# ORNL/HydraGNN

Hardware: NVIDIA H100
Metric: atoms_per_sec_training_step (higher is better)
Workload: dtype tf32

## Files before the change

hydragnn_b200/ops.py:

```python
import os

import torch
from torch.autograd.function import once_differentiable

from . import _lib

ACT_CODES = {None: 0, "none": 0, "relu": 1, "silu": 2, "tanh": 3, "sigmoid": 4, "lrelu": 5, "elu": 6, "selu": 7}
POOL_CODES = {"add": 0, "sum": 0, "mean": 1, "max": 2}


def _stream():
    return torch.cuda.current_stream().cuda_stream


def _p(t):
    return None if t is None else t.data_ptr()


def _chk(t, dtype=torch.float32):
    if t is None:
        return None
    if not t.is_cuda:
        raise RuntimeError("hydragnn_b200 ops need CUDA tensors (no CPU fallback on the hot path)")
    if t.dtype != dtype:
# ... 2 lines not shown


def _ws(nbytes, device):
    return torch.empty(max(int(nbytes), 16), dtype=torch.uint8, device=device)


class Csr:
    __slots__ = ("idx", "rowptr", "perm", "n")

    def __init__(self, idx, rowptr, perm, n):
        self.idx, self.rowptr, self.perm, self.n = idx, rowptr, perm, n


def csr_build(index64, n):
    index64 = _chk(index64, torch.int64)
    e = index64.numel()
    dev = index64.device
    idx32 = torch.empty(e, dtype=torch.int32, device=dev)
    rowptr = torch.empty(n + 1, dtype=torch.int32, device=dev)
    perm = torch.empty(e, dtype=torch.int32, device=dev)
    ws = _ws(_lib.query("hgb_csr_workspace_bytes", e, n), dev)
    _lib.call("hgb_csr_build", _p(index64), e, n, _p(idx32), _p(rowptr), _p(perm), _p(guard_flag(dev)), _p(ws), _stream())
    return Csr(idx32, rowptr, perm, n)


def csr_build_grouped(index64, n, node_ptr, edge_ptr, g):
    index64 = _chk(index64, torch.int64)
    e = index64.numel()
    dev = index64.device
    idx32 = torch.empty(e, dtype=torch.int32, device=dev)
    rowptr = torch.empty(n + 1, dtype=torch.int32, device=dev)
    perm = torch.empty(e, dtype=torch.int32, device=dev)
    ws = _ws(_lib.query("hgb_csr_grouped_workspace_bytes", e, n), dev)
    _lib.call("hgb_csr_build_grouped", _p(index64), e, n, _p(node_ptr), _p(edge_ptr), int(g), _p(idx32), _p(rowptr), _p(perm),
              _p(guard_flag(dev)), _p(ws), _stream())
    return Csr(idx32, rowptr, perm, n)


class EdgePlan:

    def __init__(self, edge_index, num_nodes, col_rowptr=None, graph_ptr=None):
        ei = _chk(edge_index, torch.int64)
        self.num_nodes, self.num_edges = int(num_nodes), int(ei.shape[1])
        if col_rowptr is not None and graph_ptr is not None and GROUPED_CSR:
            self.by_row = csr_build_grouped(ei[0], self.num_nodes, graph_ptr, col_rowptr, graph_ptr.numel() - 1)
        else:
            self.by_row = csr_build(ei[0], self.num_nodes)
        if col_rowptr is not None:
            self.by_col = Csr(ei[1].to(torch.int32), col_rowptr, torch.arange(self.num_edges, dtype=torch.int32, device=ei.device),
                              self.num_nodes)
        else:
            self.by_col = csr_build(ei[1], self.num_nodes)
        self.row, self.col = self.by_row.idx, self.by_col.idx
        self._nbr = {}

    def nbr(self, which):
        if which not in self._nbr:
            idx, perm = (self.col, self.by_row.perm) if which == "row" else (self.row, self.by_col.perm)
            out = torch.empty_like(perm)
            _lib.call("hgb_gather_i32", _p(idx), _p(perm), perm.numel(), _p(out), _stream())
            self._nbr[which] = out
        return self._nbr[which]


def graph_ptr_from_batch(batch, num_graphs):
    return csr_build(batch, num_graphs)


def exclusive_scan(x):
    x = _chk(x, torch.int32)
    out = torch.empty(x.numel() + 1, dtype=torch.int32, device=x.device)
    ws = _ws(_lib.query("hgb_exclusive_scan_workspace_bytes", x.numel()), x.device)
    _lib.call("hgb_exclusive_scan_i32", _p(x), _p(out), x.numel(), _p(ws), _stream())
    return out


GUARD_EDGE_COUNT = 1
GUARD_BAD_INDEX = 2
_GUARD = {}


def guard_flag(device):
    key = torch.device(device).index if torch.device(device).index is not None else torch.cuda.current_device()
    if key not in _GUARD:
        _GUARD[key] = torch.zeros(1, dtype=torch.int32, device=torch.device("cuda", key))
    return _GUARD[key]


def expect_count(value_i32, expected, bit=GUARD_EDGE_COUNT):
    _lib.call("hgb_expect_i32", _p(value_i32), int(expected), int(bit), _p(guard_flag(value_i32.device)), _stream())


def check_guard(device=None):
    dev = torch.device("cuda", torch.cuda.current_device()) if device is None else torch.device(device)
    word = int(guard_flag(dev).item())
    if word:
        guard_flag(dev).zero_()
        what = []
        if word & GUARD_EDGE_COUNT:
            what.append("a neighbour build produced a different edge count than the one the step was captured with")
        if word & GUARD_BAD_INDEX:
            what.append("an index vector had entries outside [0, n)")
        raise RuntimeError("hydragnn_b200 device guard tripped: " + "; ".join(what))


def raw_gather(x, idx32):
    x = _chk(x)
# ... 559 lines not shown
        gv = torch.empty_like(vec)
        _lib.call("hgb_edge_geom_bwd", _p(vec), _p(ln), ctx.eps, _p(_chk(g_vec)), _p(_chk(g_len)), _p(_chk(g_unit)),
                  plan.num_edges, _p(gv), _stream())
        g_pos = g_shift = None
        if ctx.needs_input_grad[0]:
            g_pos = raw_segment_sum(gv, plan.by_col.rowptr, plan.by_col.perm, plan.num_nodes) - \
                raw_segment_sum(gv, plan.by_row.rowptr, plan.by_row.perm, plan.num_nodes)
        if ctx.needs_input_grad[1]:
            g_shift = gv
        return g_pos, g_shift, None, None


class PainnEdgeEmbedFn(torch.autograd.Function):

    @staticmethod
    def forward(ctx, unit, ln, num_radial, cutoff):
        e = unit.shape[0]
        epack = torch.empty(e, 12, dtype=unit.dtype, device=unit.device)
        _lib.call("hgb_painn_edge_embed_fwd", _p(unit), _p(ln), e, num_radial, float(cutoff), _p(epack), _stream())
        ctx.save_for_backward(unit, ln)
        ctx.r, ctx.cutoff = num_radial, float(cutoff)
        return epack

    @staticmethod
    @once_differentiable
    def backward(ctx, g_epack):
        unit, ln = ctx.saved_tensors
        e = unit.shape[0]
        g_unit = torch.empty_like(unit)
        g_len = torch.empty_like(ln)
        _lib.call("hgb_painn_edge_embed_bwd", _p(unit), _p(ln), _p(_chk(g_epack)), e, ctx.r, ctx.cutoff, _p(g_unit), _p(g_len), _stream())
        return g_unit, g_len, None, None


class PainnMessageFn(torch.autograd.Function):

    @staticmethod
    def forward(ctx, phi, s, v, epack, wf, bf, efilt, plan, rec_row=None):
        n, f = s.shape
        r = wf.shape[1]
        phi, s, v = _chk(phi), _chk(s), _chk(v)
        s_out, v_out = torch.empty_like(s), torch.empty_like(v)
        agg = plan.by_row
        _lib.call("hgb_painn_message_fwd", _p(phi), _p(s), _p(v), _p(agg.rowptr), _p(agg.perm), _p(plan.nbr("row")), _p(epack),
                  _p(rec_row), _p(_chk(wf)), _p(_chk(bf)), _p(_chk(efilt)), n, f, r, _p(s_out), _p(v_out), _stream())
        ctx.save_for_backward(phi, v, epack, wf, bf, efilt)
        ctx.plan, ctx.use_rec = plan, rec_row is not None
        return s_out, v_out

    @staticmethod
    @once_differentiable
    def backward(ctx, gs_out, gv_out):
        phi, v, epack, wf, bf, efilt = ctx.saved_tensors
        plan = ctx.plan
        n, f = gs_out.shape
        r = wf.shape[1]
        gs_out, gv_out = _chk(gs_out), _chk(gv_out)
        need_edge = ctx.needs_input_grad[3]
        gphi, gv = torch.empty_like(phi), torch.empty_like(v)
        gwf, gbf = torch.empty_like(wf), torch.empty_like(bf)
        cpl = 2 if (f >= 64 and f % 2 == 0) else 1
        multi = f > 32 * cpl
        g_epack = (torch.zeros_like(epack) if multi else torch.empty_like(epack)) if need_edge else None
        g_ef = torch.empty_like(efilt) if efilt is not None else None
        nbytes = _lib.query("hgb_painn_message_bwd_workspace_bytes", n, f, r)
        ws = _ws(nbytes, phi.device)
        src = plan.by_col
        rec_col = None
        if ctx.use_rec:
            cache = plan.__dict__.setdefault("_rec_col", {})
            key = epack.data_ptr()
            if key not in cache:
                cache.clear()
                cache[key] = painn_edge_records(epack, plan, "col")
            rec_col = cache[key]
        _lib.call("hgb_painn_message_bwd", _p(gs_out), _p(gv_out), _p(phi), _p(v), _p(src.rowptr), _p(src.perm), _p(plan.nbr("col")),
                  _p(epack), _p(rec_col), _p(wf), _p(bf), _p(efilt), n, f, r, _p(gphi), _p(gv), _p(gwf), _p(gbf), _p(g_epack), _p(g_ef),
                  _p(ws), nbytes, _stream())
        return gphi, gs_out, gv, g_epack, gwf, gbf, g_ef, None, None


def painn_edge_records(epack, plan, which):
    csr = plan.by_row if which == "row" else plan.by_col
    rec = torch.empty(plan.num_edges, 16, dtype=epack.dtype, device=epack.device)
    _lib.call("hgb_painn_edge_records", _p(epack.detach()), _p(csr.perm), _p(plan.nbr(which)), plan.num_edges, _p(rec), _stream())
    return rec


def raw_linear(x2, w, b, code=0, param=0.0, want_z=False):
    m, k = x2.shape
    n = w.shape[0]
    y = torch.empty(m, n, dtype=x2.dtype, device=x2.device)
    z = torch.empty_like(y) if want_z else None
    if gemm3_ok(x2, w, y, m, n, k, False, True):
        _lib.call("hgb_gemm3", _p(x2), _p(w), _p(y), m, n, k, 0, 1, x2.stride(0), w.stride(0), n, 0, _p(b), code, float(param), _p(z), None,
                  _stream())
        return y, z
    _lib.call("hgb_linear_fwd", _p(x2), _p(w), _p(b), m, n, k, x2.stride(0), w.stride(0), code, float(param), _p(y), _p(z), _stream())
    return y, z


def raw_act_bwd(dy, y, z, code, param=0.0):
    dz = torch.empty_like(dy)
    _lib.call("hgb_act_bwd", _p(dy), _p(y), _p(z), dy.numel(), code, float(param), _p(dz), _stream())
    return dz


class PainnUpdateFn(torch.autograd.Function):

    @staticmethod
    def forward(ctx, s, v, uw, ub, vw, vb, w1, b1, w2, b2, last):
        n, f = s.shape
        s, v = _chk(s), _chk(v)
        w1, b1, w2, b2 = [_chk(t) for t in (w1, b1, w2, b2)]
        v2 = v.reshape(3 * n, f)
        wuv, buv = torch.cat([uw, vw], dim=0).contiguous(), torch.cat([ub, vb], dim=0).contiguous()
        y_uv, _ = linear_fwd_dispatch(v2, wuv, buv)
        uv, vv, ld = y_uv, y_uv[:, f:], 2 * f
        mlp_in = torch.empty(n, 2 * f, dtype=s.dtype, device=s.device)
        _lib.call("hgb_painn_update_pre_fwd", _p(vv), ld, _p(s), n, f, _p(mlp_in), _stream())
        h, z1, deriv = linear_fwd_dispatch_ex(mlp_in, w1, b1, ACT_CODES["silu"], 0.0, want_z=True, z_deriv=True)
        a, _ = linear_fwd_dispatch(h, w2, b2)
        ctx.z1_code = ACT_DERIV if deriv else ACT_CODES["silu"]
        s_out = torch.empty_like(s)
        v_out = None if last else torch.empty_like(v)
        _lib.call("hgb_painn_update_post_fwd", _p(a), _p(uv), _p(vv), ld, _p(s), _p(v), n, f, int(last), _p(s_out), _p(v_out), _stream())
        ctx.save_for_backward(v2, y_uv, mlp_in, z1, h, a, wuv, w1, w2)
        ctx.last = bool(last)
        ctx.tc = _TC["enabled"]
        ctx.leaves = ([uw, ub, vw, vb], [w1, b1], [w2, b2])
        if last:
            return s_out, s_out.new_zeros(0)
# ... 682 lines not shown
```

hydragnn_b200/stacks.py:

```python
import os

import torch
import torch.nn.functional as F
from torch import nn

from . import ops
from .ops import GatherRows, LinearAct, MatMul, SegmentSum


def activation_function_selection(name):
    table = {"relu": nn.ReLU, "selu": nn.SELU, "elu": nn.ELU, "sigmoid": nn.Sigmoid,
             "lrelu_01": lambda: nn.LeakyReLU(0.1), "lrelu_025": lambda: nn.LeakyReLU(0.25),
             "lrelu_05": lambda: nn.LeakyReLU(0.5)}
    if name == "prelu":
        raise ValueError("activation 'prelu' (a learnable slope) is not supported by the b200 engine")
    if name not in table:
        raise ValueError("Unknown activation function: " + str(name))
    return table[name]()


def _act_code(mod):
    if isinstance(mod, nn.ReLU):
        return "relu", 0.0
    if isinstance(mod, nn.SiLU):
# ... 154 lines not shown
            return self._forward_fused(x, coord, plan, edge_shifts, higher_order, cache)
        if higher_order:
            vec = GatherRows.apply(coord, plan.by_col) - GatherRows.apply(coord, plan.by_row)
            if edge_shifts is not None:
                vec = vec + edge_shifts
            radial = torch.linalg.norm(vec, dim=-1, keepdim=True)
            coord_diff = vec / (radial + 1.0)
        else:
            _, radial, coord_diff = ops.EdgeGeomFn.apply(coord, edge_shifts, plan, 1.0)
        lin0, fin = self.edge_mlp[0], x.shape[1]
        w0 = lin0.weight
        lin = ops.linear_any_order if higher_order else ops.linear_act
        h = GatherRows.apply(lin(x, w0[:, :fin], None), plan.by_row) + GatherRows.apply(lin(x, w0[:, fin:2 * fin], None), plan.by_col)
        h = h + radial * w0[:, 2 * fin] + lin0.bias
        if edge_attr is not None:
            h = h + lin(edge_attr, w0[:, 2 * fin + 1:], None)
        m = run_mlp(self.edge_mlp[2:], self.edge_mlp[1](h), higher_order)
        if self.equivariant:
            trans = torch.clamp(coord_diff * run_mlp(self.coord_mlp, m, higher_order), min=-100, max=100)
            cnt = (plan.by_row.rowptr[1:] - plan.by_row.rowptr[:-1]).clamp(min=1).to(trans.dtype)
            coord = coord + SegmentSum.apply(trans, plan.by_row) / cnt[:, None]
        agg = SegmentSum.apply(m, plan.by_row)
        out = run_mlp(self.node_mlp, torch.cat([x, agg], dim=1), higher_order)
        return out, coord


class PainnMessage(nn.Module):
    def __init__(self, node_size, num_radial, cutoff, edge_dim=None):
        super().__init__()
        self.node_size, self.num_radial, self.cutoff, self.edge_dim = node_size, num_radial, cutoff, edge_dim
        self.scalar_message_mlp = nn.Sequential(nn.Linear(node_size, node_size), nn.SiLU(),
                                                nn.Linear(node_size, node_size * 3))
        self.filter_layer = nn.Linear(num_radial, node_size * 3)
        if edge_dim is not None:
            self.edge_filter = nn.Sequential(nn.Linear(edge_dim, node_size), nn.SiLU(),
                                             nn.Linear(node_size, node_size * 3))

    def forward(self, s, v, plan, geom, edge_attr=None, higher_order=False):
        f = self.node_size
        if higher_order:
            diff, dist = geom["unit"], geom["len"]
            n = torch.arange(1, self.num_radial + 1, device=dist.device)
            rbf = torch.sin(dist * n * torch.pi / self.cutoff) / dist
            fcut = torch.where(dist < self.cutoff, 0.5 * (torch.cos(torch.pi * dist / self.cutoff) + 1.0),
                               torch.zeros_like(dist))
            w = ops.linear_any_order(rbf, self.filter_layer.weight, self.filter_layer.bias) * fcut
            if edge_attr is not None:
                w = w * run_mlp(self.edge_filter, edge_attr, True)
            phi = run_mlp(self.scalar_message_mlp, s, True)
            fo = w * GatherRows.apply(phi, plan.by_col)
            g_v, g_e, m_s = torch.split(fo, f, dim=1)
            m_v = GatherRows.apply(v, plan.by_col) * g_v.unsqueeze(1) + g_e.unsqueeze(1) * (diff / dist).unsqueeze(-1)
            return s + SegmentSum.apply(m_s, plan.by_row), v + SegmentSum.apply(m_v, plan.by_row)
        phi = run_mlp(self.scalar_message_mlp, s)
        efilt = run_mlp(self.edge_filter, edge_attr) if edge_attr is not None else None
        if "rec_row" not in geom and self.node_size % 64 == 0:
            geom["rec_row"] = ops.painn_edge_records(geom["epack"], plan, "row")
        return ops.PainnMessageFn.apply(phi, s, v, geom["epack"], self.filter_layer.weight, self.filter_layer.bias, efilt, plan,
                                        geom.get("rec_row"))


class PainnUpdate(nn.Module):
    def __init__(self, node_size, last_layer=False):
        super().__init__()
        self.update_U = nn.Linear(node_size, node_size)
        self.update_V = nn.Linear(node_size, node_size)
        self.last_layer = last_layer
        self.update_mlp = nn.Sequential(nn.Linear(node_size * 2, node_size), nn.SiLU(),
                                        nn.Linear(node_size, node_size * (2 if last_layer else 3)))

    def forward(self, s, v, higher_order=False):
        f = v.shape[-1]
        if higher_order:
            uv = ops.linear_any_order(v, self.update_U.weight, self.update_U.bias)
            vv = ops.linear_any_order(v, self.update_V.weight, self.update_V.bias)
            a = run_mlp(self.update_mlp, torch.cat([torch.linalg.norm(vv, dim=1), s], dim=1), True)
            inner = (uv * vv).sum(dim=1)
            if self.last_layer:
                a_sv, a_ss = torch.split(a, f, dim=1)
                return s + a_sv * inner + a_ss, None
            a_vv, a_sv, a_ss = torch.split(a, f, dim=1)
            return s + a_sv * inner + a_ss, v + a_vv.unsqueeze(1) * uv
        if f == 1 and ops.SCALAR_UPDATE:
            fn = ops.PainnUpdateScalarFn
        else:
            fn = ops.PainnUpdateTcFn if ops.painn_update_tc_ok(s, v) else ops.PainnUpdateFn
        s_out, v_out = fn.apply(s, v, self.update_U.weight, self.update_U.bias, self.update_V.weight,
                                               self.update_V.bias, self.update_mlp[0].weight, self.update_mlp[0].bias,
                                               self.update_mlp[2].weight, self.update_mlp[2].bias, self.last_layer)
        return s_out, (None if self.last_layer else v_out)


class EGNNConv(nn.Module):
    def __init__(self, egcl):
        super().__init__()
        self.module_0 = egcl

    def forward(self, inv_node_feat, equiv_node_feat, plan, edge_attr=None, edge_shifts=None, geom=None, higher_order=False):
        x, pos = self.module_0(inv_node_feat, equiv_node_feat, plan, edge_attr, edge_shifts, higher_order, cache=geom)
        return x, pos


class PainnConv(nn.Module):
    def __init__(self, msg, upd, node_embed_out, vec_embed_out):
        super().__init__()
        self.module_0, self.module_1, self.module_2 = msg, upd, node_embed_out
        if vec_embed_out is not None:
            self.module_3 = vec_embed_out
        self.last = vec_embed_out is None

# ... 390 lines not shown
```

include/hgb.h:

```cpp
#ifndef HGB_H
#define HGB_H

#include <stdint.h>

#ifdef __cplusplus
extern "C" {
#endif

typedef void* hgb_stream_t;

#define HGB_OK 0
#define HGB_EINVAL (-1)
#define HGB_ECUDA (-2)
#define HGB_ECAPACITY (-3)

#define HGB_ACT_DERIV 100
#define HGB_ACT_NONE 0
#define HGB_ACT_RELU 1
#define HGB_ACT_SILU 2
#define HGB_ACT_TANH 3
#define HGB_ACT_SIGMOID 4
#define HGB_ACT_LRELU 5
#define HGB_ACT_ELU 6
#define HGB_ACT_SELU 7
// ... 69 lines not shown
int64_t hgb_gemm_workspace_bytes(int32_t m, int32_t n, int32_t k, int32_t trans_a);
int hgb_linear_fwd(const float* x, const float* w, const float* b, int32_t m, int32_t n, int32_t k,
                   int64_t ldx, int64_t ldw, int32_t act, float act_param, float* y, float* z,
                   hgb_stream_t stream);
int hgb_linear_smallk_supported(int32_t n, int32_t k);
int hgb_linear_smallk_fwd(const float* x, int64_t ldx, const float* w, int64_t ldw, const float* b, int32_t m,
                          int32_t n, int32_t k, int32_t act, float act_param, float* y, float* z,
                          hgb_stream_t stream);
int hgb_linear_smallk_bwd(const float* dy, const float* y, const float* z, const float* x, int64_t ldx,
                          const float* w, int64_t ldw, int32_t m, int32_t n, int32_t k, int32_t act,
                          float act_param, float* dx, float* dw, int64_t lddw, float* db, void* workspace,
                          hgb_stream_t stream);
int64_t hgb_linear_smallk_bwd_workspace_bytes(int32_t m, int32_t n, int32_t k);

int hgb_tc_linear_supported(int32_t m, int32_t n_out, int32_t k_red);
int hgb_tc_linear(const float* a, int64_t lda, const float* w, int64_t ldw, int32_t trans_b, const float* bias,
                  int32_t m, int32_t n_out, int32_t k_red, int32_t act, float act_param, float* y, float* z,
                  const float* addend, const float* gsrc, int32_t gact, int32_t exact, hgb_stream_t stream);
int hgb_tc_wgrad(const float* dz, int64_t lddz, const float* x, int64_t ldx, int32_t m, int32_t n_out,
                 int32_t k_out, float* dw, int64_t lddw, float* db, int32_t accumulate, int32_t exact,
                 void* workspace, int64_t workspace_bytes, hgb_stream_t stream);
int64_t hgb_tc_wgrad_workspace_bytes(int32_t n_out, int32_t k_out);
int hgb_act_bwd(const float* dy, const float* y, const float* z, int64_t count, int32_t act,
                float act_param, float* dz, hgb_stream_t stream);
int hgb_act_deriv(const float* x, int64_t count, int32_t act, float act_param, int32_t order,
                  float* out, hgb_stream_t stream);
int hgb_colsum(const float* x, int32_t m, int32_t n, float* out, void* workspace, hgb_stream_t stream);
int64_t hgb_colsum_workspace_bytes(int32_t m, int32_t n);


int hgb_edge_geom_fwd(const float* pos, const int32_t* row, const int32_t* col, const float* shifts,
                      int64_t e, float eps, float* vec, float* len, float* unit, hgb_stream_t stream);
int hgb_edge_geom_bwd(const float* vec, const float* len, float eps, const float* g_vec_in,
                      const float* g_len, const float* g_unit, int64_t e, float* g_vec,
                      hgb_stream_t stream);
int hgb_painn_edge_embed_fwd(const float* unit, const float* len, int64_t e, int32_t r, float cutoff,
                             float* epack, hgb_stream_t stream);
int hgb_painn_edge_embed_bwd(const float* unit, const float* len, const float* g_epack, int64_t e, int32_t r,
                             float cutoff, float* g_unit, float* g_len, hgb_stream_t stream);


int hgb_painn_message_fwd(const float* phi, const float* s, const float* v, const int32_t* rowptr,
                          const int32_t* perm, const int32_t* nbr, const float* epack, const float* rec,
                          const float* wf, const float* bf, const float* efilt, int32_t n, int32_t f, int32_t r,
                          float* s_out, float* v_out, hgb_stream_t stream);
int hgb_painn_edge_records(const float* epack, const int32_t* perm, const int32_t* nbr, int64_t e, float* rec,
                           hgb_stream_t stream);
int hgb_painn_message_bwd(const float* gs_out, const float* gv_out, const float* phi, const float* v,
                          const int32_t* rowptr_src, const int32_t* perm_src, const int32_t* nbr_agg,
                          const float* epack, const float* rec, const float* wf, const float* bf, const float* efilt, int32_t n,
                          int32_t f, int32_t r, float* gphi, float* gv, float* gwf, float* gbf, float* g_epack,
                          float* g_efilt, void* workspace, int64_t workspace_bytes, hgb_stream_t stream);
int64_t hgb_painn_message_bwd_workspace_bytes(int32_t n, int32_t f, int32_t r);

int hgb_painn_update_pre_fwd(const float* vv, int64_t ld, const float* s, int32_t n, int32_t f, float* mlp_in,
                             hgb_stream_t stream);
int hgb_painn_update_post_fwd(const float* a, const float* uv, const float* vv, int64_t ld, const float* s,
                              const float* v, int32_t n, int32_t f, int32_t last, float* s_out,
                              float* v_out, hgb_stream_t stream);
int hgb_painn_update_post_bwd_a(const float* gs_out, const float* gv_out, const float* uv,
                                const float* vv, int64_t ld, int32_t n, int32_t f, int32_t last, float* ga,
                                hgb_stream_t stream);
int hgb_painn_update_bwd(const float* gs_out, const float* gv_out, const float* g_mlp_in,
                         const float* a, const float* uv, const float* vv, int64_t ld, const float* mlp_in,
                         int32_t n, int32_t f, int32_t last, float* guv, float* gvv, float* gs,
                         float* gv, hgb_stream_t stream);
int hgb_painn_update_tc_fwd(const float* v, const float* s, const float* wuv, const float* buv, int32_t n,
                            float* mlp_in, float* inner, hgb_stream_t stream);
int hgb_painn_update_tc_post(const float* v, const float* s, const float* a, const float* inner, const float* wuv,
                             const float* buv, int32_t n, int32_t last, float* s_out, float* v_out, hgb_stream_t stream);
int hgb_painn_update_tc_bwd_a(const float* v, const float* gs_out, const float* gv_out, const float* inner,
                              const float* wuv, const float* buv, int32_t n, int32_t last, float* ga, hgb_stream_t stream);
int hgb_painn_update_tc_bwd(const float* v, const float* gs_out, const float* gv_out, const float* g_mlp_in,
                            const float* a, const float* mlp_in, const float* wuv, const float* buv, int32_t n,
                            int32_t last, float* g_uv, float* gs, float* gv, hgb_stream_t stream);


int hgb_mha_fwd(const float* qkv, int32_t n, int32_t f, int32_t heads, float* out, float* lse,
                hgb_stream_t stream);
int hgb_mha_bwd(const float* qkv, const float* out, const float* lse, const float* gout, int32_t n, int32_t f,
                int32_t heads, float* gqkv, hgb_stream_t stream);

int32_t hgb_mha_tc_supported(int32_t f, int32_t heads);
int hgb_mha_tc_fwd(const float* qkv, int32_t n, int32_t f, int32_t heads, int32_t exact, float* out, float* lse,
                   hgb_stream_t stream);
int hgb_mha_tc_bwd(const float* qkv, const float* out, const float* lse, const float* gout, int32_t n, int32_t f,
                   int32_t heads, int32_t exact, float* delta_ws, float* gqkv, hgb_stream_t stream);

int hgb_mace_tp_path(int32_t mode, const float* p0, const float* p1, const float* p2, const float* cg, int64_t e, int32_t f,
                     int32_t ni, int32_t nj, int32_t nk, float* out, hgb_stream_t stream);
int hgb_mace_chan_contract(int32_t mode, const float* p0, const float* p1, int64_t n, int32_t f, int32_t p, int32_t ni,
                           float* out, hgb_stream_t stream);

int hgb_mace_edge_mix(int32_t mode, const float* src, int64_t ld, const float* eattr, int64_t e, int32_t f, int32_t d, float c,
                      float* out, hgb_stream_t stream);

int hgb_mace_edge_embed_fwd(const float* pos, const int32_t* row, const int32_t* col, const float* shifts, int64_t e, int32_t lmax,
                            int32_t num_bessel, float r_max, float p, float* sh, float* radial, hgb_stream_t stream);
int hgb_mace_edge_embed_bwd(const float* pos, const int32_t* row, const int32_t* col, const float* shifts, const float* g_sh,
                            const float* g_radial, int64_t e, int32_t lmax, int32_t num_bessel, float r_max, float p, float* g_vec,
                            hgb_stream_t stream);

int hgb_grouped_linear(const float* x, int64_t ldx, const float* w, const float* bias, const int32_t* rowptr, int32_t groups,
                       int32_t m, int32_t n, int32_t k, int32_t trans_w, int32_t act, float act_param, float* y, float* z,
                       hgb_stream_t stream);
int hgb_grouped_wgrad(const float* dy, const float* x, int64_t ldx, const int32_t* rowptr, int32_t groups, int32_t m, int32_t n,
// ... 88 lines not shown
```

profiles/kbench.py:

```python
import os, sys, json
sys.path.insert(0, os.path.dirname(os.path.dirname(os.path.abspath(__file__))))
import torch
import hydragnn_b200 as hb
from hydragnn_b200 import ops
from hydragnn_b200.stacks import Base
from hydragnn_b200.synthetic import ARCH, make_samples

dev = torch.device("cuda")
flush = torch.empty(256 * 1024 * 1024, dtype=torch.uint8, device=dev)


def timeit(fn, iters=10, warm=3):
    ts = []
    for it in range(iters + warm):
        flush.zero_()
        a, b = torch.cuda.Event(enable_timing=True), torch.cuda.Event(enable_timing=True)
        a.record(); fn(); b.record(); torch.cuda.synchronize()
        if it >= warm:
            ts.append(a.elapsed_time(b))
    return sum(ts) / len(ts)


def tc_linear_calls(n):
    silu, tanh, deriv = ops.ACT_CODES["silu"], ops.ACT_CODES["tanh"], ops.ACT_DERIV
# ... 1 lines not shown
             ("fwd 64->192", n, 64, 192, False, 0, False, 0, False, False),
             ("fwd 64->128 (3N rows)", 3 * n, 64, 128, False, 0, False, 0, False, False),
             ("fwd 128->64 silu z=silu'", n, 128, 64, False, silu, True, deriv, False, False),
             ("fwd 64->128", n, 64, 128, False, 0, False, 0, False, False),
             ("fwd 64->64 tanh", n, 64, 64, False, tanh, False, 0, False, False),
             ("dgrad 64->64 gsrc=silu'", n, 64, 64, True, 0, False, deriv, False, True),
             ("dgrad 64->192 gsrc=silu'", n, 192, 64, True, 0, False, deriv, False, True),
             ("dgrad 128->64 gsrc=silu'", n, 64, 128, True, 0, False, deriv, False, True),
             ("dgrad 64->64 gsrc=tanh", n, 64, 64, True, 0, False, tanh, False, True),
             ("dgrad 64->128 (3N rows) +addend", 3 * n, 128, 64, True, 0, False, 0, True, False),
             ("dgrad 64->128 plain", n, 128, 64, True, 0, False, 0, False, False)]
    res = {}
    for name, m, k, no, tb, act, want_z, gact, has_add, has_g in calls:
        a = torch.randn(m, k, device=dev)
        w = torch.randn(k, no, device=dev) if tb else torch.randn(no, k, device=dev)
        bias = None if tb else torch.randn(no, device=dev)
        add = torch.randn(m, no, device=dev) if has_add else None
        g = torch.rand(m, no, device=dev) if has_g else None
        t = timeit(lambda: ops.raw_tc_linear(a, w, tb, bias, no, k, act, 0.0, want_z, addend=add, gsrc=g, gact=gact))
        nbytes = 4 * m * (k + no * (1 + int(want_z) + int(has_add) + int(has_g)))
        res["tc_linear %s m=%d (ms | GB/s)" % (name, m)] = (round(t, 4), round(nbytes / t / 1e6, 1))
    return res


def painn_update_calls(n, f=64):
    from hydragnn_b200.stacks import PainnUpdate
    units = {("fused", True): (19, 44), ("fused", False): (25, 56), ("unfused", True): (32, 58), ("unfused", False): (40, 72)}
    U = n * f * 4
    res = {}
    overlap = ops.WGRAD_OVERLAP
    ops.WGRAD_OVERLAP = False
    try:
        for last in (True, False):
            upd = PainnUpdate(f, last).to(dev)
            params = [upd.update_U.weight, upd.update_U.bias, upd.update_V.weight, upd.update_V.bias, upd.update_mlp[0].weight,
                      upd.update_mlp[0].bias, upd.update_mlp[2].weight, upd.update_mlp[2].bias]
            s = torch.randn(n, f, device=dev, requires_grad=True)
            v = torch.randn(n, 3, f, device=dev, requires_grad=True)
            for kind, fn in (("fused", ops.PainnUpdateTcFn), ("unfused", ops.PainnUpdateFn)):
                with ops.tensor_cores(True):
                    so, vo = fn.apply(s, v, *params, last)
                    outs = (so,) if last else (so, vo)
                    grads = tuple(torch.randn_like(o) for o in outs)
                    t_f = timeit(lambda: fn.apply(s, v, *params, last))
                    t_b = timeit(lambda: torch.autograd.grad(outs, [s, v] + params, grads, retain_graph=True))
                uf, ub = units[(kind, last)]
                res["painn_update %s last=%s fwd (ms | GB/s | U)" % (kind, last)] = (round(t_f, 4), round(uf * U / t_f / 1e6, 1), uf)
                res["painn_update %s last=%s bwd (ms | GB/s | U)" % (kind, last)] = (round(t_b, 4), round(ub * U / t_b / 1e6, 1), ub)
    finally:
        ops.WGRAD_OVERLAP = overlap
    return res


G = 16384
b = make_samples("qm9_painn", G).to(dev); b._num_graphs = G
if os.environ.get("KBENCH_ONLY") == "tc_linear":
    print(json.dumps(tc_linear_calls(b.pos.shape[0]), indent=1)); sys.exit(0)
if os.environ.get("KBENCH_ONLY") == "painn_update":
    print(json.dumps(painn_update_calls(b.pos.shape[0]), indent=1)); sys.exit(0)
b = hb.get_radius_graph(7.0, 5)(b)
plan = Base.plan_for(b)
n, e, f, r = plan.num_nodes, plan.num_edges, 64, 5
_, ln, unit = ops.EdgeGeomFn.apply(b.pos, None, plan, 1e-9)
epack = ops.PainnEdgeEmbedFn.apply(unit, ln, r, 7.0)
s, v, phi = torch.randn(n, f, device=dev), torch.randn(n, 3, f, device=dev), torch.randn(n, 3 * f, device=dev)
wf, bf = torch.randn(3 * f, r, device=dev), torch.randn(3 * f, device=dev)
out = {}
rec = ops.painn_edge_records(epack, plan, "row")
out["painn_message_fwd F=64 (ms)"] = timeit(lambda: ops.PainnMessageFn.apply(phi, s, v, epack, wf, bf, None, plan, rec))
out["painn_edge_records (ms)"] = timeit(lambda: ops.painn_edge_records(epack, plan, "row"))
sr, vr, pr = s.clone().requires_grad_(True), v.clone().requires_grad_(True), phi.clone().requires_grad_(True)
so, vo = ops.PainnMessageFn.apply(pr, sr, vr, epack, wf.requires_grad_(True), bf.requires_grad_(True), None, plan, rec)
gs, gv = torch.randn_like(so), torch.randn_like(vo)
out["painn_message_bwd F=64 (ms)"] = timeit(lambda: torch.autograd.grad((so, vo), (pr, sr, vr, wf, bf), (gs, gv), retain_graph=True))
so2, vo2 = ops.PainnMessageFn.apply(pr, sr, vr, epack, wf, bf, None, plan, None)
out["painn_message_bwd generic F=64 (ms)"] = timeit(lambda: torch.autograd.grad((so2, vo2), (pr, sr, vr, wf, bf), (gs, gv), retain_graph=True))
if os.environ.get("KBENCH_ONLY") == "painn":
    print(json.dumps(out, indent=1)); sys.exit(0)
alg_f = e * (6 * f * 4 + 8 + 48) + n * (8 * f * 4 + 4)
out["painn_message_fwd GB/s algorithmic"] = alg_f / out["painn_message_fwd F=64 (ms)"] / 1e6
for (m, k, nn_) in [(n, 64, 64), (n, 64, 192), (3 * n, 64, 64), (n, 128, 64), (n, 192, 64)]:
    x, w, bb = torch.randn(m, k, device=dev), torch.randn(nn_, k, device=dev), torch.randn(nn_, device=dev)
    t = timeit(lambda: ops.raw_tc_linear(x, w, False, bb, nn_, k))
    out["tc_linear m=%d k=%d n=%d (ms | GB/s)" % (m, k, nn_)] = (t, m * (k + nn_) * 4 / t / 1e6)
out.update(tc_linear_calls(n))
for (m, nn_, k) in [(n, 64, 64), (n, 192, 64), (3 * n, 64, 64)]:
    dz, x = torch.randn(m, nn_, device=dev), torch.randn(m, k, device=dev)
    t = timeit(lambda: ops.raw_tc_wgrad(dz, x))
    out["tc_wgrad m=%d n=%d k=%d (ms | GB/s)" % (m, nn_, k)] = (t, m * (k + nn_) * 4 / t / 1e6)
print(json.dumps(out, indent=1))
```

Baseline: 40.87 million.

## Fuse PaiNN scalar message MLP into warp-specialized wgmma message kernel

Adds a Hopper kernel that runs the two-layer SiLU scalar message MLP with TF32 wgmma on per-graph node tiles. Separate warps gather over neighbour edges out of shared memory, with TMA/bulk loads, mbarrier double buffering and L2 prefetch. This removes the separate MLP launches and the global round trip of phi for small molecular graphs. A tile-packing kernel groups whole graphs into tiles of up to 32 nodes, and the backward reuses saved h/zd together with the existing message backward. In exchange it adds much complexity, a large shared-memory footprint with one block per SM, and extra stores of h and zd.

```diff
diff --git a/hydragnn_b200/csrc/hgb_painn_msg_tc.cu b/hydragnn_b200/csrc/hgb_painn_msg_tc.cu
--- /dev/null
+++ b/hydragnn_b200/csrc/hgb_painn_msg_tc.cu
@@ -0,0 +1,368 @@
+#include "hgb_tc.cuh"
+
+namespace {
+
+constexpr int MF = 64;
+constexpr int MF3 = 3 * MF;
+constexpr int MM = 64;
+constexpr int MT = 32;
+constexpr int MSG_THREADS = 384;
+constexpr int GATHER_WARPS = MSG_THREADS / 32 - 4;
+constexpr uint32_t SZ_W1 = MF * MF * 4;
+constexpr uint32_t SZ_W2 = MF3 * MF * 4;
+constexpr uint32_t SZ_A = MM * MF * 4;
+constexpr uint32_t SZ_ROWS = MT * MF3 * 4;
+constexpr int REC_CAP = 384;
+constexpr uint32_t SZ_BUF = 2 * SZ_ROWS + REC_CAP * 64;
+constexpr size_t MSG_SMEM = 1024 + SZ_W1 + SZ_W2 + SZ_A + 2 * (size_t)SZ_BUF + 4 * (MF + MF3) + 6 * 8;
+
+struct MsgParams {
+  const float* s;
+  const float* v;
+  const int32_t* rowptr;
+  const float* rec;
+  const float *w1, *b1, *w2, *b2, *wf, *bf;
+  const int32_t* tile_ptr;
+  const int32_t* tile_count;
+  int n, r;
+  float* h;
+  float* zd;
+  float* phi;
+  float* s_out;
+  float* v_out;
+};
+
+__device__ __forceinline__ void bulk_g2s(void* dst, const void* src, uint32_t bytes, uint64_t* bar) {
+  asm volatile("cp.async.bulk.shared::cluster.global.mbarrier::complete_tx::bytes [%0], [%1], %2, [%3];" ::"r"(smem_u32(dst)), "l"(src),
+               "r"(bytes), "r"(smem_u32(bar))
+               : "memory");
+}
+__device__ __forceinline__ void prefetch_l2(const void* p, uint32_t bytes) {
+  if (bytes) asm volatile("cp.async.bulk.prefetch.L2.global [%0], %1;" ::"l"(p), "r"(bytes) : "memory");
+}
+
+__device__ __forceinline__ void stage_weight(uint8_t* sB, const float* w, int rows, int k) {
+  for (int i = threadIdx.x; i < rows * k; i += blockDim.x) {
+    const int r = i / k, c = i - r * k;
+    *reinterpret_cast<float*>(sB + kmajor_sw128_off(r, c, rows)) = __ldg(w + i);
+  }
+}
+
+__device__ __forceinline__ void mlp_chunk(const MsgParams& p, uint8_t* sA, const uint8_t* sW1, const uint8_t* sW2, const float* sb1,
+                                          const float* sb2, int row0, int rows, float* phi, float* phi_g) {
+  const int tid = threadIdx.x, wq = tid >> 5, lane = tid & 31;
+  const uint32_t a_u = smem_u32(sA), w1_u = smem_u32(sW1), w2_u = smem_u32(sW2);
+  const int rb = 16 * wq + (lane >> 2), cq = 2 * (lane & 3);
+  {
+    float acc[32];
+#pragma unroll
+    for (int j = 0; j < 32; ++j) acc[j] = 0.f;
+    fence_regs<32>(acc);
+    wgmma_fence();
+#pragma unroll
+    for (int kb = 0; kb < 2; ++kb)
+#pragma unroll
+      for (int k4 = 0; k4 < 4; ++k4)
+        wgmma_tf32<2>(acc, make_desc(a_u + kb * 8192 + k4 * 32), make_desc(w1_u + kb * MF * 128 + k4 * 32));
+    wgmma_commit();
+    wgmma_wait<0>();
+    fence_regs<32>(acc);
+    named_bar_sync(1, 128);
+#pragma unroll
+    for (int i = 0; i < 8; ++i)
+#pragma unroll
+      for (int hh = 0; hh < 2; ++hh) {
+        const int r = rb + 8 * hh, col = 8 * i + cq;
+        float hv[2], zv[2];
+#pragma unroll
+        for (int e = 0; e < 2; ++e) {
+          float x = acc[4 * i + 2 * hh + e] + sb1[col + e];
+          const float sg = __fdividef(1.f, 1.f + __expf(-x));
+          x *= sg;
+          zv[e] = fmaf(x, 1.f - sg, sg);
+          hv[e] = x;
+        }
+        *reinterpret_cast<float2*>(sA + kmajor_sw128_off(r, col, MM)) = make_float2(hv[0], hv[1]);
+        if (r < rows) {
+          const int64_t o = (int64_t)(row0 + r) * MF + col;
+          *reinterpret_cast<float2*>(p.h + o) = make_float2(hv[0], hv[1]);
+          *reinterpret_cast<float2*>(p.zd + o) = make_float2(zv[0], zv[1]);
+        }
+      }
+    fence_proxy_async();
+    named_bar_sync(1, 128);
+  }
+  float acc[96];
+#pragma unroll
+  for (int j = 0; j < 96; ++j) acc[j] = 0.f;
+  fence_regs<96>(acc);
+  wgmma_fence();
+#pragma unroll
+  for (int kb = 0; kb < 2; ++kb)
+#pragma unroll
+    for (int k4 = 0; k4 < 4; ++k4)
+      wgmma_tf32<6>(acc, make_desc(a_u + kb * 8192 + k4 * 32), make_desc(w2_u + kb * MF3 * 128 + k4 * 32));
+  wgmma_commit();
+  wgmma_wait<0>();
+  fence_regs<96>(acc);
+#pragma unroll
+  for (int i = 0; i < 24; ++i)
+#pragma unroll
+    for (int hh = 0; hh < 2; ++hh) {
+      const int r = rb + 8 * hh, col = 8 * i + cq;
+      if (r < rows) {
+        const float2 o = make_float2(acc[4 * i + 2 * hh] + sb2[col], acc[4 * i + 2 * hh + 1] + sb2[col + 1]);
+        *reinterpret_cast<float2*>(phi + (size_t)r * MF3 + col) = o;
+        if (phi_g) *reinterpret_cast<float2*>(phi_g + (int64_t)(row0 + r) * MF3 + col) = o;
+      }
+    }
+  named_bar_sync(1, 128);
+}
+
+template <int RT, bool SMEM>
+__device__ __forceinline__ void gather_nodes(const MsgParams& p, int gw, int i0, int i1, int base, const float* phi, const float* v,
+                                             const float4* srec, int rec_lo, bool staged) {
+  const int lane = threadIdx.x & 31;
+  const int cc = lane * 2;
+  float wr[3][2][RT + 1];
+#pragma unroll
+  for (int a = 0; a < 3; ++a)
+#pragma unroll
+    for (int tt = 0; tt < 2; ++tt) {
+#pragma unroll
+      for (int q = 0; q < RT; ++q) wr[a][tt][q] = q < p.r ? __ldg(p.wf + (a * MF + cc + tt) * p.r + q) : 0.f;
+      wr[a][tt][RT] = __ldg(p.bf + a * MF + cc + tt);
+    }
+  const float4* rec4 = reinterpret_cast<const float4*>(p.rec);
+  int lo = 0, hi = 0;
+  if (i0 + gw < i1) { lo = __ldg(p.rowptr + i0 + gw); hi = __ldg(p.rowptr + i0 + gw + 1); }
+  for (int i = i0 + gw; i < i1; i += GATHER_WARPS) {
+    const float2 own_s = __ldg(reinterpret_cast<const float2*>(p.s + (int64_t)i * MF + cc));
+    int lo_n = 0, hi_n = 0;
+    if (i + GATHER_WARPS < i1) { lo_n = __ldg(p.rowptr + i + GATHER_WARPS); hi_n = __ldg(p.rowptr + i + GATHER_WARPS + 1); }
+    float as[2] = {0.f, 0.f}, av[3][2] = {{0.f, 0.f}, {0.f, 0.f}, {0.f, 0.f}};
+    for (int q0 = lo; q0 < hi; ++q0) {
+      float4 e0, e1, e2, e3;
+      const float4* ep = staged ? srec + (q0 - rec_lo) * 4 : rec4 + (int64_t)q0 * 4;
+      if (staged) { e0 = ep[0]; e1 = ep[1]; e2 = ep[2]; e3 = ep[3]; }
+      else { e0 = __ldg(ep); e1 = __ldg(ep + 1); e2 = __ldg(ep + 2); e3 = __ldg(ep + 3); }
+      const float rb[8] = {e0.x, e0.y, e0.z, e0.w, e1.x, e1.y, e1.z, e1.w};
+      const float fce = e2.x, d[3] = {e2.y, e2.z, e2.w};
+      const int j = __float_as_int(e3.x) - base;
+      float pv[3][2], vv[3][2];
+#pragma unroll
+      for (int a = 0; a < 3; ++a) {
+        const float* pp = phi + (size_t)j * MF3 + a * MF + cc;
+        const float* vp = v + (size_t)j * MF3 + a * MF + cc;
+        float2 x2, y2;
+        if (SMEM) { x2 = *reinterpret_cast<const float2*>(pp); y2 = *reinterpret_cast<const float2*>(vp); }
+        else { x2 = *reinterpret_cast<const float2*>(pp); y2 = __ldg(reinterpret_cast<const float2*>(vp)); }
+        pv[a][0] = x2.x; pv[a][1] = x2.y; vv[a][0] = y2.x; vv[a][1] = y2.y;
+      }
+#pragma unroll
+      for (int tt = 0; tt < 2; ++tt) {
+        float w[3];
+#pragma unroll
+        for (int a = 0; a < 3; ++a) {
+          float acc = wr[a][tt][RT] * fce;
+#pragma unroll
+          for (int q = 0; q < RT; ++q) acc = fmaf(wr[a][tt][q], rb[q], acc);
+          w[a] = acc;
+        }
+        const float gv = w[0] * pv[0][tt], ge = w[1] * pv[1][tt];
+        as[tt] = fmaf(w[2], pv[2][tt], as[tt]);
+#pragma unroll
+        for (int k = 0; k < 3; ++k) av[k][tt] = fmaf(ge, d[k], fmaf(vv[k][tt], gv, av[k][tt]));
+      }
+    }
+    *reinterpret_cast<float2*>(p.s_out + (int64_t)i * MF + cc) = make_float2(own_s.x + as[0], own_s.y + as[1]);
+#pragma unroll
+    for (int k = 0; k < 3; ++k) {
+      const float* vp = v + (size_t)(i - base) * MF3 + k * MF + cc;
+      const float2 own = SMEM ? *reinterpret_cast<const float2*>(vp) : __ldg(reinterpret_cast<const float2*>(vp));
+      *reinterpret_cast<float2*>(p.v_out + (int64_t)i * MF3 + k * MF + cc) = make_float2(own.x + av[k][0], own.y + av[k][1]);
+    }
+    lo = lo_n;
+    hi = hi_n;
+  }
+}
+
+}
+
+template <int RT>
+__global__ void __launch_bounds__(MSG_THREADS, 1) painn_message_tc_fwd_kernel(const __grid_constant__ CUtensorMap tmap_s, const MsgParams p) {
+  extern __shared__ uint8_t smem_raw[];
+  uint8_t* smem = reinterpret_cast<uint8_t*>((reinterpret_cast<uintptr_t>(smem_raw) + 1023) & ~(uintptr_t)1023);
+  uint8_t* sW1 = smem;
+  uint8_t* sW2 = sW1 + SZ_W1;
+  uint8_t* sA = sW2 + SZ_W2;
+  uint8_t* sBuf = sA + SZ_A;
+  float* sb1 = reinterpret_cast<float*>(sBuf + 2 * SZ_BUF);
+  float* sb2 = sb1 + MF;
+  uint64_t* ld = reinterpret_cast<uint64_t*>(sb2 + MF3);
+  uint64_t* full = ld + 2;
+  uint64_t* empty = full + 2;
+  uint64_t* chunk = empty + 2;
+  auto sPhi = [&](int b) { return reinterpret_cast<float*>(sBuf + (size_t)b * SZ_BUF); };
+  auto sV = [&](int b) { return reinterpret_cast<float*>(sBuf + (size_t)b * SZ_BUF + SZ_ROWS); };
+  auto sRec = [&](int b) { return reinterpret_cast<float4*>(sBuf + (size_t)b * SZ_BUF + 2 * SZ_ROWS); };
+
+  stage_weight(sW1, p.w1, MF, MF);
+  stage_weight(sW2, p.w2, MF3, MF);
+  for (int i = threadIdx.x; i < MF + MF3; i += blockDim.x) sb1[i] = i < MF ? __ldg(p.b1 + i) : __ldg(p.b2 + i - MF);
+  if (threadIdx.x == 0) {
+    for (int b = 0; b < 2; ++b) { mbar_init(ld + b, 1); mbar_init(full + b, 1); mbar_init(empty + b, GATHER_WARPS); }
+    mbar_init(chunk, 1);
+    fence_barrier_init();
+  }
+  fence_proxy_async();
+  __syncthreads();
+
+  const int ntiles = __ldg(p.tile_count);
+  if (threadIdx.x < 128) {
+    uint32_t cphase = 0;
+    int it = 0;
+    for (int t = blockIdx.x; t < ntiles; t += gridDim.x, ++it) {
+      const int b = it & 1;
+      const uint32_t use = (uint32_t)it >> 1;
+      const int n0 = __ldg(p.tile_ptr + t), n1 = __ldg(p.tile_ptr + t + 1), cnt = n1 - n0;
+      const int e0 = __ldg(p.rowptr + n0), ecnt = __ldg(p.rowptr + n1) - e0;
+      if (it >= 2) mbar_wait(empty + b, (use - 1) & 1);
+      if (cnt <= MT) {
+        if (threadIdx.x == 0) {
+          fence_proxy_async();
+          const uint32_t vb = (uint32_t)cnt * MF3 * 4, rb = ecnt <= REC_CAP ? (uint32_t)ecnt * 64 : 0;
+          mbar_expect_tx(ld + b, SZ_A + vb + rb);
+          tma_load_2d(sA, &tmap_s, ld + b, 0, n0);
+          tma_load_2d(sA + 8192, &tmap_s, ld + b, 32, n0);
+          bulk_g2s(sV(b), p.v + (int64_t)n0 * MF3, vb, ld + b);
+          if (rb) bulk_g2s(sRec(b), p.rec + (int64_t)e0 * 16, rb, ld + b);
+          const int tn = t + gridDim.x;
+          if (tn < ntiles) {
+            const int m0 = __ldg(p.tile_ptr + tn), m1 = __ldg(p.tile_ptr + tn + 1);
+            const int f0 = __ldg(p.rowptr + m0), f1 = __ldg(p.rowptr + m1);
+            prefetch_l2(p.s + (int64_t)m0 * MF, (uint32_t)(m1 - m0) * MF * 4);
+            prefetch_l2(p.v + (int64_t)m0 * MF3, (uint32_t)(m1 - m0) * MF3 * 4);
+            prefetch_l2(p.rec + (int64_t)f0 * 16, (uint32_t)(f1 - f0) * 64);
+          }
+        }
+        mbar_wait(ld + b, use & 1);
+        mlp_chunk(p, sA, sW1, sW2, sb1, sb2, n0, cnt, sPhi(b), p.phi);
+      } else {
+        if (threadIdx.x == 0) mbar_arrive(ld + b);
+        for (int c0 = n0; c0 < n1; c0 += MM) {
+          if (threadIdx.x == 0) {
+            fence_proxy_async();
+            mbar_expect_tx(chunk, SZ_A);
+            tma_load_2d(sA, &tmap_s, chunk, 0, c0);
+            tma_load_2d(sA + 8192, &tmap_s, chunk, 32, c0);
+          }
+          mbar_wait(chunk, cphase);
+          cphase ^= 1;
+          mlp_chunk(p, sA, sW1, sW2, sb1, sb2, c0, min(MM, n1 - c0), p.phi + (int64_t)c0 * MF3, nullptr);
+        }
+        __threadfence_block();
+        named_bar_sync(1, 128);
+      }
+      if (threadIdx.x == 0) mbar_arrive(full + b);
+    }
+  } else {
+    const int gw = (threadIdx.x >> 5) - 4, lane = threadIdx.x & 31;
+    int it = 0;
+    for (int t = blockIdx.x; t < ntiles; t += gridDim.x, ++it) {
+      const int b = it & 1;
+      const uint32_t use = (uint32_t)it >> 1;
+      const int n0 = __ldg(p.tile_ptr + t), n1 = __ldg(p.tile_ptr + t + 1), cnt = n1 - n0;
+      const int e0 = __ldg(p.rowptr + n0), ecnt = __ldg(p.rowptr + n1) - e0;
+      mbar_wait(ld + b, use & 1);
+      mbar_wait(full + b, use & 1);
+      if (cnt <= MT) gather_nodes<RT, true>(p, gw, n0, n1, n0, sPhi(b), sV(b), sRec(b), e0, ecnt <= REC_CAP);
+      else gather_nodes<RT, false>(p, gw, n0, n1, 0, p.phi, p.v, nullptr, 0, false);
+      __syncwarp();
+      if (lane == 0) mbar_arrive(empty + b);
+    }
+  }
+}
+
+namespace {
+
+constexpr int TILE_THREADS = 1024;
+
+__device__ __forceinline__ int pack_run(const int32_t* gp, int k0, int k1, int32_t* out) {
+  int cnt = 0, cur = 0;
+  for (int k = k0; k < k1; ++k) {
+    const int sz = gp[k + 1] - gp[k];
+    if (sz == 0) continue;
+    if (cur > 0 && cur + sz > MT) cur = 0;
+    if (cur == 0) {
+      if (out) out[cnt] = gp[k];
+      ++cnt;
+    }
+    cur = sz > MT ? 0 : cur + sz;
+  }
+  return cnt;
+}
+
+__global__ void __launch_bounds__(TILE_THREADS) painn_msg_tiles_kernel(const int32_t* __restrict__ gp, int g, int run,
+                                                                       int32_t* __restrict__ tile_ptr, int32_t* __restrict__ tile_count) {
+  __shared__ int scan[TILE_THREADS];
+  const int t = threadIdx.x;
+  const int k0 = min(g, t * run), k1 = min(g, k0 + run);
+  const int c = pack_run(gp, k0, k1, nullptr);
+  scan[t] = c;
+  __syncthreads();
+  for (int o = 1; o < TILE_THREADS; o <<= 1) {
+    const int x = t >= o ? scan[t - o] : 0;
+    __syncthreads();
+    scan[t] += x;
+    __syncthreads();
+  }
+  pack_run(gp, k0, k1, tile_ptr + scan[t] - c);
+  if (t == TILE_THREADS - 1) {
+    tile_ptr[scan[t]] = gp[g];
+    *tile_count = scan[t];
+  }
+}
+
+}
+
+extern "C" int hgb_painn_msg_tc_tiles(const int32_t* graph_ptr, int32_t g, int32_t* tile_ptr, int32_t* tile_count, hgb_stream_t stream) {
+  HGB_REQUIRE(g >= 1 && graph_ptr && tile_ptr && tile_count, "painn_msg_tc_tiles: bad arguments");
+  int run = (g + TILE_THREADS - 1) / TILE_THREADS;
+  if (run < 64) run = 64;
+  painn_msg_tiles_kernel<<<1, TILE_THREADS, 0, (cudaStream_t)stream>>>(graph_ptr, g, run, tile_ptr, tile_count);
+  HGB_LAUNCH_CHECK("painn_msg_tc_tiles");
+  return HGB_OK;
+}
+
+extern "C" int hgb_painn_message_tc_fwd(const float* s, const float* v, const int32_t* rowptr, const float* rec, const float* w1,
+                                        const float* b1, const float* w2, const float* b2, const float* wf, const float* bf,
+                                        const int32_t* tile_ptr, const int32_t* tile_count, int32_t max_tiles, int32_t n, int32_t r,
+                                        float* h, float* zd, float* phi, float* s_out, float* v_out, hgb_stream_t stream) {
+  HGB_REQUIRE(n >= 0 && r > 0 && r <= 8, "painn_message_tc_fwd: need 0 < num_radial <= 8 (got %d)", r);
+  HGB_REQUIRE(s && v && rowptr && rec && w1 && b1 && w2 && b2 && wf && bf && tile_ptr && tile_count && h && zd && phi && s_out && v_out,
+              "painn_message_tc_fwd: null pointer");
+  HGB_REQUIRE((((uintptr_t)s | (uintptr_t)v | (uintptr_t)rec | (uintptr_t)h | (uintptr_t)zd | (uintptr_t)phi | (uintptr_t)s_out |
+                (uintptr_t)v_out) & 15) == 0,
+              "painn_message_tc_fwd: operands must be 16-byte aligned");
+  if (n == 0 || max_tiles <= 0) return HGB_OK;
+  CUtensorMap tm;
+  int rc = make_tmap(&tm, s, n, MF, MF, MM, CU_TENSOR_MAP_SWIZZLE_128B);
+  if (rc) return rc;
+  MsgParams p;
+  p.s = s; p.v = v; p.rowptr = rowptr; p.rec = rec; p.w1 = w1; p.b1 = b1; p.w2 = w2; p.b2 = b2; p.wf = wf; p.bf = bf;
+  p.tile_ptr = tile_ptr; p.tile_count = tile_count; p.n = n; p.r = r; p.h = h; p.zd = zd; p.phi = phi; p.s_out = s_out;
+  p.v_out = v_out;
+  const int grid = max_tiles < HGB_NUM_SMS ? max_tiles : HGB_NUM_SMS;
+  cudaStream_t st = (cudaStream_t)stream;
+  static bool attr_done = false;
+  if (!attr_done) {
+    cudaFuncSetAttribute(painn_message_tc_fwd_kernel<5>, cudaFuncAttributeMaxDynamicSharedMemorySize, (int)MSG_SMEM);
+    cudaFuncSetAttribute(painn_message_tc_fwd_kernel<8>, cudaFuncAttributeMaxDynamicSharedMemorySize, (int)MSG_SMEM);
+    attr_done = true;
+  }
+  if (r <= 5) painn_message_tc_fwd_kernel<5><<<grid, MSG_THREADS, MSG_SMEM, st>>>(tm, p);
+  else painn_message_tc_fwd_kernel<8><<<grid, MSG_THREADS, MSG_SMEM, st>>>(tm, p);
+  HGB_LAUNCH_CHECK("painn_message_tc_fwd");
+  return HGB_OK;
+}
diff --git a/hydragnn_b200/ops.py b/hydragnn_b200/ops.py
--- a/hydragnn_b200/ops.py
+++ b/hydragnn_b200/ops.py
@@ -78,7 +78,18 @@
         else:
             self.by_col = csr_build(ei[1], self.num_nodes)
         self.row, self.col = self.by_row.idx, self.by_col.idx
+        self.graph_ptr = graph_ptr if col_rowptr is not None else None
         self._nbr = {}
+        self._tiles = None
+
+    def graph_tiles(self):
+        if self._tiles is None:
+            g = self.graph_ptr.numel() - 1
+            tile_ptr = torch.empty(g + 1, dtype=torch.int32, device=self.graph_ptr.device)
+            tile_count = torch.empty(1, dtype=torch.int32, device=self.graph_ptr.device)
+            _lib.call("hgb_painn_msg_tc_tiles", _p(self.graph_ptr), g, _p(tile_ptr), _p(tile_count), _stream())
+            self._tiles = (tile_ptr, tile_count, g)
+        return self._tiles
 
     def nbr(self, which):
         if which not in self._nbr:
@@ -744,32 +755,76 @@
     @once_differentiable
     def backward(ctx, gs_out, gv_out):
         phi, v, epack, wf, bf, efilt = ctx.saved_tensors
-        plan = ctx.plan
-        n, f = gs_out.shape
-        r = wf.shape[1]
-        gs_out, gv_out = _chk(gs_out), _chk(gv_out)
-        need_edge = ctx.needs_input_grad[3]
-        gphi, gv = torch.empty_like(phi), torch.empty_like(v)
-        gwf, gbf = torch.empty_like(wf), torch.empty_like(bf)
-        cpl = 2 if (f >= 64 and f % 2 == 0) else 1
-        multi = f > 32 * cpl
-        g_epack = (torch.zeros_like(epack) if multi else torch.empty_like(epack)) if need_edge else None
-        g_ef = torch.empty_like(efilt) if efilt is not None else None
-        nbytes = _lib.query("hgb_painn_message_bwd_workspace_bytes", n, f, r)
-        ws = _ws(nbytes, phi.device)
-        src = plan.by_col
-        rec_col = None
-        if ctx.use_rec:
-            cache = plan.__dict__.setdefault("_rec_col", {})
-            key = epack.data_ptr()
-            if key not in cache:
-                cache.clear()
-                cache[key] = painn_edge_records(epack, plan, "col")
-            rec_col = cache[key]
-        _lib.call("hgb_painn_message_bwd", _p(gs_out), _p(gv_out), _p(phi), _p(v), _p(src.rowptr), _p(src.perm), _p(plan.nbr("col")),
-                  _p(epack), _p(rec_col), _p(wf), _p(bf), _p(efilt), n, f, r, _p(gphi), _p(gv), _p(gwf), _p(gbf), _p(g_epack), _p(g_ef),
-                  _p(ws), nbytes, _stream())
+        gs_out = _chk(gs_out)
+        gphi, gv, g_epack, gwf, gbf, g_ef = painn_message_bwd(gs_out, gv_out, phi, v, epack, wf, bf, efilt, ctx.plan, ctx.use_rec,
+                                                              ctx.needs_input_grad[3])
         return gphi, gs_out, gv, g_epack, gwf, gbf, g_ef, None, None
+
+
+def painn_message_bwd(gs_out, gv_out, phi, v, epack, wf, bf, efilt, plan, use_rec, need_edge):
+    n, f = gs_out.shape
+    r = wf.shape[1]
+    gs_out, gv_out = _chk(gs_out), _chk(gv_out)
+    gphi, gv = torch.empty_like(phi), torch.empty_like(v)
+    gwf, gbf = torch.empty_like(wf), torch.empty_like(bf)
+    cpl = 2 if (f >= 64 and f % 2 == 0) else 1
+    multi = f > 32 * cpl
+    g_epack = (torch.zeros_like(epack) if multi else torch.empty_like(epack)) if need_edge else None
+    g_ef = torch.empty_like(efilt) if efilt is not None else None
+    nbytes = _lib.query("hgb_painn_message_bwd_workspace_bytes", n, f, r)
+    ws = _ws(nbytes, phi.device)
+    src = plan.by_col
+    rec_col = None
+    if use_rec:
+        cache = plan.__dict__.setdefault("_rec_col", {})
+        key = epack.data_ptr()
+        if key not in cache:
+            cache.clear()
+            cache[key] = painn_edge_records(epack, plan, "col")
+        rec_col = cache[key]
+    _lib.call("hgb_painn_message_bwd", _p(gs_out), _p(gv_out), _p(phi), _p(v), _p(src.rowptr), _p(src.perm), _p(plan.nbr("col")),
+              _p(epack), _p(rec_col), _p(wf), _p(bf), _p(efilt), n, f, r, _p(gphi), _p(gv), _p(gwf), _p(gbf), _p(g_epack), _p(g_ef),
+              _p(ws), nbytes, _stream())
+    return gphi, gv, g_epack, gwf, gbf, g_ef
+
+
+def painn_message_tc_ok(s, v, plan, edge_attr, higher_order):
+    n, f = s.shape
+    gp = plan.graph_ptr
+    return (_TC["enabled"] and f == 64 and edge_attr is None and not higher_order and gp is not None and gp.dtype == torch.int32
+            and gp.numel() >= 2 and n >= 256 and tuple(v.shape) == (n, 3, f) and s.is_cuda and v.is_cuda
+            and s.dtype == torch.float32 and v.dtype == torch.float32 and s.is_contiguous() and v.is_contiguous()
+            and s.data_ptr() % 16 == 0 and v.data_ptr() % 16 == 0 and bool(_lib.query("hgb_tc_linear_supported", n, f, f)))
+
+
+class PainnMessageTcFn(torch.autograd.Function):
+
+    @staticmethod
+    def forward(ctx, s, v, epack, w1, b1, w2, b2, wf, bf, plan, rec_row):
+        n, f = s.shape
+        ctx.leaves = ([w1, b1], [w2, b2])
+        w1, b1, w2, b2, wf, bf = [_chk(t) for t in (w1, b1, w2, b2, wf, bf)]
+        tile_ptr, tile_count, cap = plan.graph_tiles()
+        h, zd = torch.empty_like(s), torch.empty_like(s)
+        phi = torch.empty(n, 3 * f, dtype=s.dtype, device=s.device)
+        s_out, v_out = torch.empty_like(s), torch.empty_like(v)
+        _lib.call("hgb_painn_message_tc_fwd", _p(s), _p(v), _p(plan.by_row.rowptr), _p(rec_row), _p(w1), _p(b1), _p(w2), _p(b2), _p(wf),
+                  _p(bf), _p(tile_ptr), _p(tile_count), cap, n, wf.shape[1], _p(h), _p(zd), _p(phi), _p(s_out), _p(v_out), _stream())
+        ctx.save_for_backward(s, v, epack, h, zd, phi, w1, w2, wf, bf)
+        ctx.plan = plan
+        return s_out, v_out
+
+    @staticmethod
+    @once_differentiable
+    def backward(ctx, gs_out, gv_out):
+        s, v, epack, h, zd, phi, w1, w2, wf, bf = ctx.saved_tensors
+        gs_out = _chk(gs_out)
+        gphi, gv, g_epack, gwf, gbf, _ = painn_message_bwd(gs_out, gv_out, phi, v, epack, wf, bf, None, ctx.plan, True,
+                                                           ctx.needs_input_grad[2])
+        with tensor_cores(True):
+            gz1, gw2, gb2 = linear_bwd_dispatch(gphi, h, w2, dx_gsrc=zd, dx_gact=ACT_DERIV, leaves=ctx.leaves[1])
+            gs, gw1, gb1 = linear_bwd_dispatch(gz1, s, w1, dx_addend=gs_out, leaves=ctx.leaves[0])
+        return gs, gv, g_epack, gw1, gb1, gw2, gb2, gwf, gbf, None, None
 
 
 def painn_edge_records(epack, plan, which):
diff --git a/hydragnn_b200/stacks.py b/hydragnn_b200/stacks.py
--- a/hydragnn_b200/stacks.py
+++ b/hydragnn_b200/stacks.py
@@ -230,10 +230,14 @@
             g_v, g_e, m_s = torch.split(fo, f, dim=1)
             m_v = GatherRows.apply(v, plan.by_col) * g_v.unsqueeze(1) + g_e.unsqueeze(1) * (diff / dist).unsqueeze(-1)
             return s + SegmentSum.apply(m_s, plan.by_row), v + SegmentSum.apply(m_v, plan.by_row)
+        if "rec_row" not in geom and self.node_size % 64 == 0:
+            geom["rec_row"] = ops.painn_edge_records(geom["epack"], plan, "row")
+        if ops.painn_message_tc_ok(s, v, plan, edge_attr, higher_order):
+            mlp = self.scalar_message_mlp
+            return ops.PainnMessageTcFn.apply(s, v, geom["epack"], mlp[0].weight, mlp[0].bias, mlp[2].weight, mlp[2].bias,
+                                              self.filter_layer.weight, self.filter_layer.bias, plan, geom["rec_row"])
         phi = run_mlp(self.scalar_message_mlp, s)
         efilt = run_mlp(self.edge_filter, edge_attr) if edge_attr is not None else None
-        if "rec_row" not in geom and self.node_size % 64 == 0:
-            geom["rec_row"] = ops.painn_edge_records(geom["epack"], plan, "row")
         return ops.PainnMessageFn.apply(phi, s, v, geom["epack"], self.filter_layer.weight, self.filter_layer.bias, efilt, plan,
                                         geom.get("rec_row"))
 
diff --git a/include/hgb.h b/include/hgb.h
--- a/include/hgb.h
+++ b/include/hgb.h
@@ -145,6 +145,12 @@
                           int32_t f, int32_t r, float* gphi, float* gv, float* gwf, float* gbf, float* g_epack,
                           float* g_efilt, void* workspace, int64_t workspace_bytes, hgb_stream_t stream);
 int64_t hgb_painn_message_bwd_workspace_bytes(int32_t n, int32_t f, int32_t r);
+
+int hgb_painn_msg_tc_tiles(const int32_t* graph_ptr, int32_t g, int32_t* tile_ptr, int32_t* tile_count, hgb_stream_t stream);
+int hgb_painn_message_tc_fwd(const float* s, const float* v, const int32_t* rowptr, const float* rec, const float* w1,
+                             const float* b1, const float* w2, const float* b2, const float* wf, const float* bf,
+                             const int32_t* tile_ptr, const int32_t* tile_count, int32_t max_tiles, int32_t n, int32_t r,
+                             float* h, float* zd, float* phi, float* s_out, float* v_out, hgb_stream_t stream);
 
 int hgb_painn_update_pre_fwd(const float* vv, int64_t ld, const float* s, int32_t n, int32_t f, float* mlp_in,
                              hgb_stream_t stream);
diff --git a/profiles/kbench.py b/profiles/kbench.py
--- a/profiles/kbench.py
+++ b/profiles/kbench.py
@@ -77,6 +77,39 @@
     return res
 
 
+def painn_message_calls(plan, epack, f=64):
+    n = plan.num_nodes
+    U = n * f * 4
+    recu = plan.num_edges * 64 / U
+    units = {"fused": (13 + recu, 24 + recu), "unfused": (18 + recu, 26 + recu)}
+    from hydragnn_b200.stacks import PainnMessage
+    msg = PainnMessage(f, 5, 7.0).to(dev)
+    m = msg.scalar_message_mlp
+    p = [m[0].weight, m[0].bias, m[2].weight, m[2].bias, msg.filter_layer.weight, msg.filter_layer.bias]
+    s = torch.randn(n, f, device=dev, requires_grad=True)
+    v = torch.randn(n, 3, f, device=dev, requires_grad=True)
+    rec = ops.painn_edge_records(epack, plan, "row")
+
+    def fused():
+        return ops.PainnMessageTcFn.apply(s, v, epack, *p, plan, rec)
+
+    def unfused():
+        phi = ops.Mlp2Fn.apply(s, p[0], p[1], "silu", 0.0, p[2], p[3], None, 0.0)
+        return ops.PainnMessageFn.apply(phi, s, v, epack, p[4], p[5], None, plan, rec)
+
+    res = {}
+    for kind, fn in (("fused", fused), ("unfused", unfused)):
+        with ops.tensor_cores(True):
+            so, vo = fn()
+            gs, gv = torch.randn_like(so), torch.randn_like(vo)
+            t_f = timeit(fn)
+            t_b = timeit(lambda: torch.autograd.grad((so, vo), (s, v), (gs, gv), retain_graph=True))
+        uf, ub = units[kind]
+        res["painn_message %s fwd (ms | GB/s | U)" % kind] = (round(t_f, 4), round(uf * U / t_f / 1e6, 1), round(uf, 2))
+        res["painn_message %s bwd (ms | GB/s | U)" % kind] = (round(t_b, 4), round(ub * U / t_b / 1e6, 1), round(ub, 2))
+    return res
+
+
 G = 16384
 b = make_samples("qm9_painn", G).to(dev); b._num_graphs = G
 if os.environ.get("KBENCH_ONLY") == "tc_linear":
@@ -88,6 +121,8 @@
 n, e, f, r = plan.num_nodes, plan.num_edges, 64, 5
 _, ln, unit = ops.EdgeGeomFn.apply(b.pos, None, plan, 1e-9)
 epack = ops.PainnEdgeEmbedFn.apply(unit, ln, r, 7.0)
+if os.environ.get("KBENCH_ONLY") == "painn_message":
+    print(json.dumps(painn_message_calls(plan, epack.detach()), indent=1)); sys.exit(0)
 s, v, phi = torch.randn(n, f, device=dev), torch.randn(n, 3, f, device=dev), torch.randn(n, 3 * f, device=dev)
 wf, bf = torch.randn(3 * f, r, device=dev), torch.randn(3 * f, device=dev)
 out = {}
```

Result: no change. 41.34 million, median of 6 (+1.2%).
